# noc-lab/sac-expert

Hardware: NVIDIA B200
Metric: agent-updates/sec (higher is better)
Workload: dtype f32

## Files before the change

### sac_expert_b200/csrc/mlp_ws.cuh

```cuda
#pragma once
#include "tc_gemm.cuh"
#include "planes.cuh"

namespace saceo {

constexpr int WS_NEW = 16;
constexpr int WS_NEPI = WS_NEW * 32, WS_NT = WS_NEPI + 64;
constexpr int WS_NST = 3, WS_RING = WS_NST * WS_STAGE;
constexpr int WS_AUX = 49152;
constexpr int WS_PATCH1 = 32 * 32 * 4;
constexpr int WS_PATCH = WS_NEW * WS_PATCH1;
constexpr int WS_MAIN = WS_RING + WS_AUX + WS_PATCH;
constexpr int WS_BYTES = WS_MAIN + 1024 + 256;
constexpr int WS_RED = 40960;
constexpr int WS_MAXOUT = 36;
enum { WB_FULL = 0, WB_EMPTY = WS_NST, WB_XFULL = 2 * WS_NST, WB_XEMPTY, WB_D0, WB_D1, WB_AP  };

__device__ __forceinline__ void mbar_arrive(uint32_t bar) {
  asm volatile("mbarrier.arrive.shared::cta.b64 _, [%0];" ::"r"(bar) : "memory");
}
__device__ __forceinline__ void mbar_expect_tx(uint32_t bar, uint32_t bytes) {
  asm volatile("mbarrier.arrive.expect_tx.shared::cta.b64 _, [%0], %1;" ::"r"(bar), "r"(bytes) : "memory");
}
__device__ __forceinline__ void bulk_g2s(uint32_t dst, const void* src, uint32_t bytes, uint32_t bar) {
  asm volatile("cp.async.bulk.shared::cluster.global.mbarrier::complete_tx::bytes [%0], [%1], %2, [%3];"
               ::"r"(dst), "l"(src), "r"(bytes), "r"(bar) : "memory");
}
__device__ __forceinline__ void bulk_prefetch_l2(const void* src, uint32_t bytes) {
  asm volatile("cp.async.bulk.prefetch.L2.global [%0], %1;" ::"l"(src), "r"(bytes) : "memory");
}
__device__ __forceinline__ void epi_bar() { asm volatile("bar.sync 1, 512;" ::: "memory"); }
__device__ __forceinline__ uint64_t umma_desc_mn(uint32_t saddr) {
  return (uint64_t)((saddr >> 4) & 0x3FFF) | ((uint64_t)(4096 >> 4) << 16) | ((uint64_t)(1024 >> 4) << 32) |
         ((uint64_t)1 << 46) | ((uint64_t)2 << 61);
}
constexpr uint32_t WS_IDESC_FWD = (1u << 4) | (1u << 16) | ((uint32_t)(256 >> 3) << 17) | ((uint32_t)(128 >> 4) << 24);
constexpr uint32_t WS_IDESC_BWD = (1u << 4) | ((uint32_t)(128 >> 3) << 17) | ((uint32_t)(128 >> 4) << 24);

__global__ void k_planes_build(const float* __restrict__ theta, long long stride, uint8_t* __restrict__ img, int K0) {
  const int n0 = (K0 + 31) / 32, rows = n0 * 32 + 256;
  const int item = blockIdx.x * blockDim.x + threadIdx.x;
  if (item >= rows * 32) return;
  const int row = item >> 5, c8 = item & 31;
  const float* th = theta + (long long)blockIdx.y * stride;
  float x[8];
  if (row < n0 * 32) {
#pragma unroll
    for (int j = 0; j < 8; ++j) x[j] = row < K0 ? th[(long long)row * 256 + c8 * 8 + j] : 0.f;
  } else {
    const long long o = (long long)K0 * 256 + 256 + (long long)(row - n0 * 32) * 256 + c8 * 8;
#pragma unroll
    for (int j = 0; j < 8; ++j) x[j] = th[o + j];
  }
  uint4 hi, lo;
  split8<true>(x, hi, lo);
  uint8_t* dst = img + (long long)blockIdx.y * ws_image_bytes(K0) + ws_image_off(row, c8);
  *reinterpret_cast<uint4*>(dst) = hi;
  *reinterpret_cast<uint4*>(dst + 16384) = lo;
}

__device__ __forceinline__ uint32_t ws_pa(uint32_t patch, int r, int c) {
  return patch + (uint32_t)(r * 128 + ((((c >> 2) ^ (r & 7)) << 4) | ((c & 3) << 2)));
}
__device__ __forceinline__ void ws_store_rows(uint32_t patch, const uint32_t (&v)[32], float* __restrict__ G, int rbase,
                                              int rows, int col, int lane, uint32_t cs = 0, int q = 0) {
#pragma unroll
  for (int j = 0; j < 8; ++j) sts128(ws_pa(patch, lane, 4 * j), make_uint4(v[4 * j], v[4 * j + 1], v[4 * j + 2], v[4 * j + 3]));
  __syncwarp();
// ... 232 lines not shown
}
__device__ __forceinline__ void ws_split_f16(const uint32_t (&v)[32], float scale, uint32_t (&hi)[16], uint32_t (&lo)[16]) {
#pragma unroll
  for (int j = 0; j < 16; ++j) {
    const float x0 = __uint_as_float(v[2 * j]) * scale, x1 = __uint_as_float(v[2 * j + 1]) * scale;
    asm("cvt.rn.satfinite.f16x2.f32 %0, %1, %2;" : "=r"(hi[j]) : "f"(x1), "f"(x0));
    const float2 hf = __half22float2(*reinterpret_cast<const __half2*>(&hi[j]));
    asm("cvt.rn.satfinite.f16x2.f32 %0, %1, %2;" : "=r"(lo[j]) : "f"(x1 - hf.y), "f"(x0 - hf.x));
  }
}
template <int ACT>
__device__ __forceinline__ void ws_bias_act(uint32_t (&v)[32], uint32_t bias) {
#pragma unroll
  for (int j = 0; j < 8; ++j) {
    const float4 b = lds128(bias + j * 16);
    v[4 * j] = __float_as_uint(apply_act(ACT, __uint_as_float(v[4 * j]) + b.x));
    v[4 * j + 1] = __float_as_uint(apply_act(ACT, __uint_as_float(v[4 * j + 1]) + b.y));
    v[4 * j + 2] = __float_as_uint(apply_act(ACT, __uint_as_float(v[4 * j + 2]) + b.z));
    v[4 * j + 3] = __float_as_uint(apply_act(ACT, __uint_as_float(v[4 * j + 3]) + b.w));
  }
}
__device__ __forceinline__ void ws_bias_act_rt(int act, uint32_t (&v)[32], uint32_t bias) {
  if (act == ACT_RELU) ws_bias_act<ACT_RELU>(v, bias);
  else if (act == ACT_TANH) ws_bias_act<ACT_TANH>(v, bias);
  else ws_bias_act<ACT_ELU>(v, bias);
}
template <int ACT>
__device__ __forceinline__ void ws_mul_dact(uint32_t (&v)[32], const float (&aux)[32], float s) {
#pragma unroll
  for (int j = 0; j < 32; ++j) v[j] = __float_as_uint(__uint_as_float(v[j]) * s * dact_from_out(ACT, aux[j]));
}
__device__ __forceinline__ void ws_mul_dact_rt(int act, uint32_t (&v)[32], const float (&aux)[32], float s) {
  if (act == ACT_RELU) ws_mul_dact<ACT_RELU>(v, aux, s);
  else if (act == ACT_TANH) ws_mul_dact<ACT_TANH>(v, aux, s);
  else ws_mul_dact<ACT_ELU>(v, aux, s);
}
__device__ __forceinline__ float ws_row_scale(float bound) {
  if (!(bound > 0.f) || !(bound < 3.0e38f)) return 1.f;
  int e;
  frexpf(bound, &e);
  e = 10 - e;
  e = e > 120 ? 120 : (e < -120 ? -120 : e);
  return ldexpf(1.f, e);
}

struct FwdW {
  const float* X; int ldx; long long sXa, sXn;
  const float* theta; long long sTa, sTn;
  const uint8_t* planes; long long sPa, sPn;
  float* H1; float* H2; long long sHa, sHn;
  uint8_t* H1p; long long sQa, sQn;
  float* Out; int ldo; long long sOa, sOn;
  int rows, K0, nout, nnet, act0, act1;
  unsigned long long* dbg;
};
#define WS_STAMP(i) do { if (f.dbg && lane == 0) f.dbg[(size_t)(blockIdx.y * gridDim.x + blockIdx.x) * 16 + (i)] = gtime(); } while (0)

template <int NG>
__global__ void __launch_bounds__(WS_NT, 1) k_mlp_fwd_ws(FwdW f) {
  extern __shared__ uint8_t smem_raw[];
  const uint32_t sb = (smem_u32(smem_raw) + 1023u) & ~1023u;
  const uint32_t ring = sb, aux = sb + WS_RING, patch_base = aux + WS_AUX, bars = sb + WS_MAIN, tslot = bars + 8 * 16;
  auto bar = [&](int i) { return bars + 8u * (uint32_t)i; };
  const int z = blockIdx.y, agent = z / f.nnet, net = z - agent * f.nnet;
  const int row0 = blockIdx.x * TC_BM;
  const int warp = threadIdx.x >> 5, lane = threadIdx.x & 31;
  const int n0 = (f.K0 + 31) >> 5, nk64 = (f.K0 + 63) >> 6;

  if (threadIdx.x == 0) {
    for (int s = 0; s < 2 * WS_NST; ++s) mbar_init(bar(s), 1);
    mbar_init(bar(WB_XFULL), WS_NEW); mbar_init(bar(WB_XEMPTY), 1);
    mbar_init(bar(WB_D0), 1); mbar_init(bar(WB_D1), 1);
    for (int g = 0; g < 4; ++g) mbar_init(bar(WB_AP + g), 8);
    asm volatile("fence.mbarrier_init.release.cluster;" ::: "memory");
  }
  if (warp == WS_NEW + 1) {
    asm volatile("tcgen05.alloc.cta_group::1.sync.aligned.shared::cta.b32 [%0], %1;" ::"r"(tslot), "n"(512) : "memory");
    asm volatile("tcgen05.relinquish_alloc_permit.cta_group::1.sync.aligned;" ::: "memory");
  }
  asm volatile("tcgen05.fence::before_thread_sync;" ::: "memory");
  __syncthreads();
  asm volatile("tcgen05.fence::after_thread_sync;" ::: "memory");
  const uint32_t tmem = lds_u32(tslot);
  const uint32_t tP = tmem, tQ = tmem + 256;

  if (warp == WS_NEW) {
    if (lane == 0) {
      const uint8_t* img = f.planes + agent * f.sPa + net * f.sPn;
      const int total = n0 + 8;
      for (int it = 0; it < total; ++it) {
        const int s = it % WS_NST;
        mbar_wait(bar(WB_EMPTY + s), (uint32_t)(((it / WS_NST) & 1) ^ 1));
        mbar_expect_tx(bar(WB_FULL + s), WS_STAGE);
        bulk_g2s(ring + s * WS_STAGE, img + (long long)it * WS_STAGE, WS_STAGE, bar(WB_FULL + s));
        if (it == WS_NST - 1)
          for (int j = WS_NST; j < total; ++j) bulk_prefetch_l2(img + (long long)j * WS_STAGE, WS_STAGE);
      }
      WS_STAMP(11);
    }
  } else if (warp == WS_NEW + 1) {
    if (lane == 0) {
      int it = 0;
      for (int sl = 0; sl < nk64; ++sl) {
        mbar_wait(bar(WB_XFULL), (uint32_t)(sl & 1));
        asm volatile("tcgen05.fence::after_thread_sync;" ::: "memory");
        for (int hh = 0; hh < 2 && sl * 2 + hh < n0; ++hh, ++it) {
          const int s = it % WS_NST;
          mbar_wait(bar(WB_FULL + s), (uint32_t)((it / WS_NST) & 1));
          asm volatile("tcgen05.fence::after_thread_sync;" ::: "memory");
          const uint32_t st = ring + s * WS_STAGE;
#pragma unroll
          for (int kk = 0; kk < 2; ++kk) {
            const uint32_t ka = (uint32_t)(hh * 2 + kk) * 32, kb = (uint32_t)kk * 2048;
            umma_f16(tP, umma_desc(aux + ka), umma_desc_mn(st + kb), WS_IDESC_FWD, (it | kk) ? 1u : 0u);
            umma_f16(tP, umma_desc(aux + ka), umma_desc_mn(st + 16384 + kb), WS_IDESC_FWD, 1u);
            umma_f16(tP, umma_desc(aux + 16384 + ka), umma_desc_mn(st + kb), WS_IDESC_FWD, 1u);
          }
          umma_commit(bar(WB_EMPTY + s));
        }
        umma_commit(bar(WB_XEMPTY));
      }
      umma_commit(bar(WB_D0));
      WS_STAMP(8);
      for (int g = 0; g < 4; ++g) {
        mbar_wait(bar(WB_AP + g), 0);
        asm volatile("tcgen05.fence::after_thread_sync;" ::: "memory");
        if (g == 3) WS_STAMP(9);
        for (int tt = 0; tt < 2; ++tt, ++it) {
          const int t = 2 * g + tt, s = it % WS_NST;
          mbar_wait(bar(WB_FULL + s), (uint32_t)((it / WS_NST) & 1));
          asm volatile("tcgen05.fence::after_thread_sync;" ::: "memory");
          const uint32_t st = ring + s * WS_STAGE;
#pragma unroll
          for (int kk = 0; kk < 2; ++kk) {
            const uint32_t ta_hi = tP + 32 * t + 8 * kk, ta_lo = ta_hi + 16, kb = (uint32_t)kk * 2048;
            umma_f16_ts(tQ, ta_hi, umma_desc_mn(st + kb), WS_IDESC_FWD, (t | kk) ? 1u : 0u);
            umma_f16_ts(tQ, ta_hi, umma_desc_mn(st + 16384 + kb), WS_IDESC_FWD, 1u);
            umma_f16_ts(tQ, ta_lo, umma_desc_mn(st + kb), WS_IDESC_FWD, 1u);
          }
          umma_commit(bar(WB_EMPTY + s));
        }
      }
      umma_commit(bar(WB_D1));
      WS_STAMP(10);
    }
  } else {
    const int q = warp & 3, cg = warp >> 2;
    const uint32_t lane_addr = (uint32_t)(q * 32) << 16;
    const uint32_t patch = patch_base + (uint32_t)warp * WS_PATCH1;
    const int rbase = row0 + q * 32, grow = rbase + lane;
    const float* __restrict__ X = f.X + agent * f.sXa + net * f.sXn;
    const float* __restrict__ th = f.theta + agent * f.sTa + net * f.sTn;
    const long long ob0 = (long long)f.K0 * FW_H, oW1 = ob0 + FW_H, ob1 = oW1 + (long long)FW_H * FW_H,
                    oW2 = ob1 + FW_H, ob2 = oW2 + (long long)FW_H * f.nout;
    float* H1 = f.H1 ? f.H1 + agent * f.sHa + net * f.sHn : nullptr;
    float* H2 = f.H2 ? f.H2 + agent * f.sHa + net * f.sHn : nullptr;
    float* Out = f.Out + agent * f.sOa + net * f.sOn;
    if (warp == 0) WS_STAMP(0);
    const int np = (f.nout + 3) & ~3;
    const uint32_t cb0 = aux + WS_RED + 2048, cb1 = cb0 + 1024, cw2 = cb1 + 1024, cb2 = cw2 + 1024;
    if (threadIdx.x < FW_H) {
      const int t = threadIdx.x;
      asm volatile("st.shared.f32 [%0], %1;" ::"r"(cb0 + t * 4), "f"(__ldg(th + ob0 + t)) : "memory");
      asm volatile("st.shared.f32 [%0], %1;" ::"r"(cb1 + t * 4), "f"(__ldg(th + ob1 + t)) : "memory");
      if (f.nout == 1) asm volatile("st.shared.f32 [%0], %1;" ::"r"(cw2 + t * 4), "f"(__ldg(th + oW2 + t)) : "memory");
      if (t < f.nout) asm volatile("st.shared.f32 [%0], %1;" ::"r"(cb2 + t * 4), "f"(__ldg(th + ob2 + t)) : "memory");
    }
    {
      Slab<TC_BM, WS_NEPI> sx;
      sx.init(X, f.ldx, 1, row0, f.rows);
      for (int sl = 0; sl < nk64; ++sl) {
        sx.ld(sl * 64, f.K0);
        if (sl > 0) mbar_wait(bar(WB_XEMPTY), (uint32_t)((sl - 1) & 1));
        sx.template st<true>(aux, aux + 16384);
        asm volatile("fence.proxy.async.shared::cta;" ::: "memory");
        __syncwarp();
        if (lane == 0) mbar_arrive(bar(WB_XFULL));
      }
    }
    epi_bar();
    if (warp == 0) WS_STAMP(1);
    mbar_wait(bar(WB_D0), 0);
    asm volatile("tcgen05.fence::after_thread_sync;" ::: "memory");
    if (warp == 0) WS_STAMP(2);
#pragma unroll 1
    for (int c = 0; c < 2; ++c) {
      const int kg = 2 * c + (cg >> 1), col = kg * 64 + (cg & 1) * 32;
      uint32_t v[32];
      tmem_ld32(tP + lane_addr + (uint32_t)col, v);
      ws_bias_act_rt(f.act0, v, cb0 + col * 4);
      ws_split_store(tP + lane_addr + (uint32_t)col, v, 1.f);
      {
        asm volatile("tcgen05.wait::st.sync.aligned;" ::: "memory");
        asm volatile("tcgen05.fence::before_thread_sync;" ::: "memory");
        __syncwarp();
        if (lane == 0) mbar_arrive(bar(WB_AP + kg));
      }
      if (f.H1p) {
#pragma unroll
        for (int j = 0; j < 8; ++j) sts128(ws_pa(patch, lane, 4 * j), make_uint4(v[4 * j], v[4 * j + 1], v[4 * j + 2], v[4 * j + 3]));
        __syncwarp();
        ws_store_planes_p(patch, f.H1p + agent * f.sQa + net * f.sQn, rbase, f.rows, col, lane);
        __syncwarp();
      } else if (H1) { ws_store_rows(patch, v, H1, rbase, f.rows, col, lane); __syncwarp(); }
    }
    if (warp == 0) WS_STAMP(3);
    if (f.nout > 1 && threadIdx.x < FW_H) {
      float w2r[NG * 16];
      ws_load_wrow<NG * 16>(th + oW2, threadIdx.x, f.nout, w2r);
      ws_store_wrow<NG * 16>(aux, threadIdx.x, np, w2r);
    }
    epi_bar();
    if (warp == 0) WS_STAMP(4);
    mbar_wait(bar(WB_D1), 0);
    asm volatile("tcgen05.fence::after_thread_sync;" ::: "memory");
    if (warp == 0) WS_STAMP(5);
    float acc[NG * 16];
#pragma unroll
    for (int i = 0; i < NG * 16; ++i) acc[i] = 0.f;
    float qacc = 0.f;
    auto head_chunk = [&](uint32_t (&v)[32], int col) {
      if (f.nout == 1) {
#pragma unroll
        for (int j = 0; j < 8; ++j) {
          const float4 t4 = lds128(cw2 + (uint32_t)(col + 4 * j) * 4);
          qacc = fmaf(__uint_as_float(v[4 * j]), t4.x, qacc); qacc = fmaf(__uint_as_float(v[4 * j + 1]), t4.y, qacc);
          qacc = fmaf(__uint_as_float(v[4 * j + 2]), t4.z, qacc); qacc = fmaf(__uint_as_float(v[4 * j + 3]), t4.w, qacc);
        }
      } else {
#pragma unroll
        for (int jj = 0; jj < 32; ++jj) {
          const float h = __uint_as_float(v[jj]);
          const uint32_t wrow = aux + (uint32_t)((col + jj) * np) * 4;
#pragma unroll
          for (int g4 = 0; g4 < NG * 4; ++g4) {
            if (g4 * 4 < np) {
              const float4 w = lds128(wrow + g4 * 16);
              acc[4 * g4] = fmaf(h, w.x, acc[4 * g4]); acc[4 * g4 + 1] = fmaf(h, w.y, acc[4 * g4 + 1]);
              acc[4 * g4 + 2] = fmaf(h, w.z, acc[4 * g4 + 2]); acc[4 * g4 + 3] = fmaf(h, w.w, acc[4 * g4 + 3]);
            }
          }
        }
      }
    };
#pragma unroll 1
    for (int c = 0; c < 2; ++c) {
      const int col = cg * 64 + c * 32;
      uint32_t v[32];
      tmem_ld32(tQ + lane_addr + (uint32_t)col, v);
      ws_bias_act_rt(f.act1, v, cb1 + col * 4);
      if (H2) { ws_store_rows(patch, v, H2, rbase, f.rows, col, lane); __syncwarp(); }
      head_chunk(v, col);
    }
    if (warp == 0) WS_STAMP(6);
    const uint32_t red = aux + WS_RED;
    if (f.nout == 1) {
      if (cg > 0) asm volatile("st.shared.f32 [%0], %1;" ::"r"(red + (uint32_t)((cg - 1) * TC_BM + q * 32 + lane) * 4), "f"(qacc) : "memory");
      epi_bar();
      if (cg == 0 && grow < f.rows) {
        const uint32_t r = red + (uint32_t)(q * 32 + lane) * 4;
        Out[(long long)grow * f.ldo] = ((qacc + lds32(r)) + (lds32(r + TC_BM * 4) + lds32(r + 2 * TC_BM * 4))) + lds32(cb2);
      }
    } else {
#pragma unroll
      for (int r0 = 0; r0 < NG * 16; r0 += 32) {
        if (r0 < f.nout) {
          if (cg > 0) {
#pragma unroll
            for (int cc = 0; cc < 32; ++cc)
              if (r0 + cc < NG * 16) asm volatile("st.shared.f32 [%0], %1;" ::"r"(patch + (uint32_t)(lane * 32 + ((cc + lane) & 31)) * 4), "f"(acc[(r0 + cc) < NG * 16 ? r0 + cc : 0]) : "memory");
          }
          epi_bar();
          if (cg == 0 && grow < f.rows) {
#pragma unroll
            for (int cc = 0; cc < 32; ++cc) {
              if (r0 + cc < NG * 16 && r0 + cc < f.nout) {
                const uint32_t o = (uint32_t)(lane * 32 + ((cc + lane) & 31)) * 4;
                const float p1 = lds32(patch_base + (uint32_t)(warp + 4) * WS_PATCH1 + o), p2 = lds32(patch_base + (uint32_t)(warp + 8) * WS_PATCH1 + o),
                            p3 = lds32(patch_base + (uint32_t)(warp + 12) * WS_PATCH1 + o);
                Out[(long long)grow * f.ldo + r0 + cc] = ((acc[(r0 + cc) < NG * 16 ? r0 + cc : 0] + p1) + (p2 + p3)) + lds32(cb2 + (uint32_t)(r0 + cc) * 4);
              }
            }
          }
          if (r0 + 32 < f.nout) epi_bar();
        }
      }
    }
    if (warp == 0) WS_STAMP(7);
  }
  asm volatile("tcgen05.fence::before_thread_sync;" ::: "memory");
  __syncthreads();
  if (warp == WS_NEW + 1) {
    asm volatile("tcgen05.dealloc.cta_group::1.sync.aligned.b32 %0, %1;" ::"r"(tmem), "n"(512) : "memory");
  }
}

struct BwdW {
  const float* dOut; int ldd; long long sDa, sDn; int kout;
  const float* theta; long long sTa, sTn; int K0, nout;
  const uint8_t* planes; long long sPa, sPn;
  const float* H1; const float* H2; long long sHa, sHn;
  float* dH2; float* dH1;
  uint8_t* dH2p; long long sQa, sQn;
  uint8_t* dH1p;
  const uint8_t* H1p;
  float* dXa; int s_cols, a_cols; long long sXa, sXn;
  int rows, nnet, act0, act1;
  float* dbpart;
  unsigned long long* dbg;
};

template <int NG, int NA, int MODE>
__global__ void __launch_bounds__(WS_NT, 1) k_mlp_bwd_ws(BwdW f) {
  extern __shared__ uint8_t smem_raw[];
  const uint32_t sb = (smem_u32(smem_raw) + 1023u) & ~1023u;
  const uint32_t ring = sb, aux = sb + WS_RING, patch_base = aux + WS_AUX, bars = sb + WS_MAIN, tslot = bars + 8 * 16;
  const uint32_t cs2 = aux + WS_RED, cs1 = cs2 + 4096;
  auto bar = [&](int i) { return bars + 8u * (uint32_t)i; };
  const int z = blockIdx.y, agent = z / f.nnet, net = z - agent * f.nnet;
  const int row0 = blockIdx.x * TC_BM;
  const int warp = threadIdx.x >> 5, lane = threadIdx.x & 31;
  const int n0 = (f.K0 + 31) >> 5;

  if (threadIdx.x == 0) {
    for (int s = 0; s < 2 * WS_NST; ++s) mbar_init(bar(s), 1);
    mbar_init(bar(WB_D0), 1); mbar_init(bar(WB_D1), 1);
    for (int g = 0; g < 4; ++g) mbar_init(bar(WB_AP + g), 8);
    asm volatile("fence.mbarrier_init.release.cluster;" ::: "memory");
    asm volatile("st.shared.u32 [%0], %1;" ::"r"(aux + WS_RED - 256), "r"(0u) : "memory");
  }
  if (warp == WS_NEW + 1) {
    asm volatile("tcgen05.alloc.cta_group::1.sync.aligned.shared::cta.b32 [%0], %1;" ::"r"(tslot), "n"(512) : "memory");
    asm volatile("tcgen05.relinquish_alloc_permit.cta_group::1.sync.aligned;" ::: "memory");
  }
  asm volatile("tcgen05.fence::before_thread_sync;" ::: "memory");
  __syncthreads();
  asm volatile("tcgen05.fence::after_thread_sync;" ::: "memory");
  const uint32_t tmem = lds_u32(tslot);
  const uint32_t tP = tmem, tQ = tmem + 256;

  if (warp == WS_NEW) {
    if (lane == 0) {
      const uint8_t* w1 = f.planes + agent * f.sPa + net * f.sPn + (long long)n0 * WS_STAGE;
      for (int it = 0; it < 8; ++it) {
        const int h = it >> 2, sj = it & 3, s = it % WS_NST;
        mbar_wait(bar(WB_EMPTY + s), (uint32_t)(((it / WS_NST) & 1) ^ 1));
        mbar_expect_tx(bar(WB_FULL + s), WS_STAGE);
        for (int pl = 0; pl < 2; ++pl)
          for (int tt = 0; tt < 4; ++tt)
// ... 384 lines not shown
    epi_bar();
    if (threadIdx.x == 0) mbar_arrive(bar(2 * DW0_NST + 1));
  }
  if (warp == WS_NEW + 1) {
    if (lane == 0) {
      mbar_wait(bar(2 * DW0_NST + 1), 0);
      asm volatile("tcgen05.fence::after_thread_sync;" ::: "memory");
      for (int it = 0; it < nst; ++it) {
        const int s = it % DW0_NST;
        mbar_wait(bar(s), (uint32_t)((it / DW0_NST) & 1));
        asm volatile("tcgen05.fence::after_thread_sync;" ::: "memory");
        const uint32_t sa = xs + (uint32_t)it * DW0_XST, sbb = ring + s * WS_STAGE;
#pragma unroll
        for (int kk = 0; kk < 2; ++kk) {
          const uint32_t ko = (uint32_t)kk * 2048;
          const uint32_t a_hi = sa + ko, a_lo = a_hi + 4096, b_hi = sbb + ko, b_lo = b_hi + 16384, acc = (it | kk) ? 1u : 0u;
          umma_f16(tmem, umma_desc_mn(a_hi), umma_desc_mn(b_hi), DW_IDESC, acc);
          umma_f16(tmem, umma_desc_mn(a_hi), umma_desc_mn(b_lo), DW_IDESC, 1u);
          umma_f16(tmem, umma_desc_mn(a_lo), umma_desc_mn(b_hi), DW_IDESC, 1u);
        }
        umma_commit(bar(DW0_NST + s));
      }
      umma_commit(bar(2 * DW0_NST));
    }
  } else if (warp < WS_NEW) {
    const int q = warp & 3, cg = warp >> 2;
    if (q * 32 < f.in) {
      const uint32_t lane_addr = (uint32_t)(q * 32) << 16;
      const uint32_t patch = ring + (uint32_t)warp * WS_PATCH1;
      float* G = f.G + agent * f.sGa + net * f.sGn;
      mbar_wait(bar(2 * DW0_NST), 0);
      asm volatile("tcgen05.fence::after_thread_sync;" ::: "memory");
#pragma unroll 1
      for (int c = 0; c < 2; ++c) {
        const int col = cg * 64 + c * 32;
        uint32_t v[32];
        tmem_ld32(tmem + lane_addr + (uint32_t)col, v);
        ws_store_rows(patch, v, G, q * 32, f.in, col, lane);
        __syncwarp();
      }
    }
  }
  asm volatile("tcgen05.fence::before_thread_sync;" ::: "memory");
  __syncthreads();
  if (warp == WS_NEW + 1) {
    asm volatile("tcgen05.dealloc.cta_group::1.sync.aligned.b32 %0, %1;" ::"r"(tmem), "n"(256) : "memory");
  }
}
static inline bool dw0_planes_eligible(int in, int rows, int ldx, const float* X, long long sXa, long long sXn) {
  return in >= 1 && in <= 64 && ((rows + 31) >> 5) <= DW0_MAXST && (ldx % 4) == 0 && (reinterpret_cast<uintptr_t>(X) & 15) == 0 &&
         (sXa % 4) == 0 && (sXn % 4) == 0;
}

static inline cudaError_t mlp_ws_init() {
  static bool done_dev[64] = {};
  int dev_ = 0; cudaGetDevice(&dev_);
  bool& done = done_dev[dev_ & 63];
  if (done) return cudaSuccess;
  cudaError_t e;
#define WS_ATTR(K) e = cudaFuncSetAttribute(K, cudaFuncAttributeMaxDynamicSharedMemorySize, WS_BYTES); if (e) return e;
  WS_ATTR(k_mlp_fwd_ws<1>) WS_ATTR(k_mlp_fwd_ws<2>) WS_ATTR(k_mlp_fwd_ws<3>)
  WS_ATTR((k_mlp_bwd_ws<0, 0, 0>)) WS_ATTR((k_mlp_bwd_ws<0, 1, 0>)) WS_ATTR((k_mlp_bwd_ws<0, 2, 0>))
  WS_ATTR((k_mlp_bwd_ws<1, 0, 0>)) WS_ATTR((k_mlp_bwd_ws<2, 0, 0>)) WS_ATTR((k_mlp_bwd_ws<3, 0, 0>))
  WS_ATTR((k_mlp_bwd_ws<0, 0, 1>)) WS_ATTR((k_mlp_bwd_ws<1, 0, 1>)) WS_ATTR((k_mlp_bwd_ws<0, 1, 2>))
#undef WS_ATTR
  e = cudaFuncSetAttribute(k_dw_planes, cudaFuncAttributeMaxDynamicSharedMemorySize, DW_BYTES); if (e) return e;
  e = cudaFuncSetAttribute(k_dw0_planes, cudaFuncAttributeMaxDynamicSharedMemorySize, DW0_BYTES); if (e) return e;
  done = true;
  return cudaSuccess;
}
static inline bool mlp_fwd_ws_eligible(int h1, int h2, int nout, int K0, const float* theta, long long sTa, long long sTn) {
  return h1 == FW_H && h2 == FW_H && nout >= 1 && nout <= WS_MAXOUT && K0 >= 1 &&
         ((reinterpret_cast<uintptr_t>(theta) & 15) == 0) && ((sTa & 3) == 0) && ((sTn & 3) == 0);
}
static inline cudaError_t mlp_fwd_ws_launch(const FwdW& f, int nagents, cudaStream_t st) {
  dim3 grid((f.rows + TC_BM - 1) / TC_BM, nagents * f.nnet);
  if (f.nout <= 16) k_mlp_fwd_ws<1><<<grid, WS_NT, WS_BYTES, st>>>(f);
  else if (f.nout <= 32) k_mlp_fwd_ws<2><<<grid, WS_NT, WS_BYTES, st>>>(f);
  else k_mlp_fwd_ws<3><<<grid, WS_NT, WS_BYTES, st>>>(f);
  return cudaPeekAtLastError();
}
static inline bool mlp_bwd_ws_eligible(int h1, int h2, int kout, int nout, bool want_dxa, int a_cols, const float* theta, long long sTa,
                                       long long sTn) {
  if (!(h1 == FW_H && h2 == FW_H && kout >= 1 && kout <= WS_MAXOUT && kout <= nout)) return false;
  if (want_dxa && (kout != 1 || a_cols < 1 || a_cols > 32)) return false;
  return ((reinterpret_cast<uintptr_t>(theta) & 15) == 0) && ((sTa & 3) == 0) && ((sTn & 3) == 0);
}
static inline cudaError_t mlp_bwd_ws_launch(const BwdW& f, int nagents, cudaStream_t st) {
  dim3 grid((f.rows + TC_BM - 1) / TC_BM, nagents * f.nnet);
  const int ng = f.kout == 1 ? 0 : (f.kout + 15) / 16, na = f.dXa ? (f.a_cols + 15) / 16 : 0;
  const bool m1 = f.H1p && f.dH2p && f.dH1p && !f.dH2 && !f.dH1, m2 = f.H1p && !f.dH2p && !f.dH1p && !f.dH2 && !f.dH1;
  if (ng == 0 && na == 0 && m1) k_mlp_bwd_ws<0, 0, 1><<<grid, WS_NT, WS_BYTES, st>>>(f);
  else if (ng == 1 && na == 0 && m1) k_mlp_bwd_ws<1, 0, 1><<<grid, WS_NT, WS_BYTES, st>>>(f);
  else if (ng == 0 && na == 1 && m2) k_mlp_bwd_ws<0, 1, 2><<<grid, WS_NT, WS_BYTES, st>>>(f);
  else if (ng == 0 && na == 0) k_mlp_bwd_ws<0, 0, 0><<<grid, WS_NT, WS_BYTES, st>>>(f);
  else if (ng == 0 && na == 1) k_mlp_bwd_ws<0, 1, 0><<<grid, WS_NT, WS_BYTES, st>>>(f);
  else if (ng == 0) k_mlp_bwd_ws<0, 2, 0><<<grid, WS_NT, WS_BYTES, st>>>(f);
  else if (ng == 1) k_mlp_bwd_ws<1, 0, 0><<<grid, WS_NT, WS_BYTES, st>>>(f);
  else if (ng == 2) k_mlp_bwd_ws<2, 0, 0><<<grid, WS_NT, WS_BYTES, st>>>(f);
  else k_mlp_bwd_ws<3, 0, 0><<<grid, WS_NT, WS_BYTES, st>>>(f);
  return cudaPeekAtLastError();
}

}
```

Measured before the change: 127,000.

## Make forward warp-specialized MLP kernel persistent with cross-item prefetch and overlap

Turns the forward MLP kernel into a persistent kernel with one block per SM that loops over (agent, net, row-tile) work items. Barrier phases carry across items so the TMA producer and MMA warp can start the next item's weight planes and layer-1 GEMM while the epilogue warps finish the current one. Biases are double-buffered through cp.async, the W2 head matrix is staged into extra shared memory ahead of time, and the next item's X rows are prefetched into L2. This is meant to remove per-block launch, setup and TMEM-allocation cost and to hide load latency, at the price of more shared memory and more involved phase tracking.

```diff
diff --git a/sac_expert_b200/csrc/mlp_ws.cuh b/sac_expert_b200/csrc/mlp_ws.cuh
--- a/sac_expert_b200/csrc/mlp_ws.cuh
+++ b/sac_expert_b200/csrc/mlp_ws.cuh
@@ -13,7 +13,11 @@
 constexpr int WS_MAIN = WS_RING + WS_AUX + WS_PATCH;
 constexpr int WS_BYTES = WS_MAIN + 1024 + 256;
 constexpr int WS_RED = 40960;
+constexpr int WS_FWD_MAIN = WS_MAIN + 16384, WS_FWD_BYTES = WS_FWD_MAIN + 1024 + 256;
+constexpr int WS_CB1 = 36864;
+static_assert(WS_FWD_BYTES <= 232448, "fused forward kernel exceeds the per-block shared-memory limit");
 constexpr int WS_MAXOUT = 36;
+static_assert(WS_CB1 >= 256 * WS_MAXOUT * 4 && WS_CB1 + 3072 + WS_MAXOUT * 4 <= WS_RED, "constant buffer overlaps AUX neighbours");
 enum { WB_FULL = 0, WB_EMPTY = WS_NST, WB_XFULL = 2 * WS_NST, WB_XEMPTY, WB_D0, WB_D1, WB_AP  };
 
 __device__ __forceinline__ void mbar_arrive(uint32_t bar) {
@@ -352,20 +356,33 @@
   uint8_t* H1p; long long sQa, sQn;
   float* Out; int ldo; long long sOa, sOn;
   int rows, K0, nout, nnet, act0, act1;
+  int nitems;
   unsigned long long* dbg;
 };
-#define WS_STAMP(i) do { if (f.dbg && lane == 0) f.dbg[(size_t)(blockIdx.y * gridDim.x + blockIdx.x) * 16 + (i)] = gtime(); } while (0)
+#define WS_STAMP(i) do { if (f.dbg && lane == 0) f.dbg[(size_t)item * 16 + (i)] = gtime(); } while (0)
+__device__ __forceinline__ void cp_async4(uint32_t dst, const float* src) {
+  asm volatile("cp.async.ca.shared.global [%0], [%1], 4;" ::"r"(dst), "l"(src) : "memory");
+}
+__device__ __forceinline__ void cp_async_commit() { asm volatile("cp.async.commit_group;" ::: "memory"); }
+__device__ __forceinline__ void ws_x_prefetch(const float* __restrict__ X, int ldx, int row0, int rows, int K0) {
+  const int r = row0 + (int)(threadIdx.x & (TC_BM - 1));
+  if (r >= rows) return;
+  const float* p = X + (long long)r * ldx;
+  for (int c = (int)(threadIdx.x >> 7) * 32; c < K0; c += (WS_NEPI / TC_BM) * 32) asm volatile("prefetch.global.L2 [%0];" ::"l"(p + c));
+  if ((threadIdx.x >> 7) == 0) asm volatile("prefetch.global.L2 [%0];" ::"l"(p + K0 - 1));
+}
 
 template <int NG>
 __global__ void __launch_bounds__(WS_NT, 1) k_mlp_fwd_ws(FwdW f) {
+  constexpr bool W2OWN = NG == 1;
   extern __shared__ uint8_t smem_raw[];
   const uint32_t sb = (smem_u32(smem_raw) + 1023u) & ~1023u;
-  const uint32_t ring = sb, aux = sb + WS_RING, patch_base = aux + WS_AUX, bars = sb + WS_MAIN, tslot = bars + 8 * 16;
+  const uint32_t ring = sb, aux = sb + WS_RING, patch_base = aux + WS_AUX, bars = sb + WS_FWD_MAIN, tslot = bars + 8 * 16;
   auto bar = [&](int i) { return bars + 8u * (uint32_t)i; };
-  const int z = blockIdx.y, agent = z / f.nnet, net = z - agent * f.nnet;
-  const int row0 = blockIdx.x * TC_BM;
   const int warp = threadIdx.x >> 5, lane = threadIdx.x & 31;
-  const int n0 = (f.K0 + 31) >> 5, nk64 = (f.K0 + 63) >> 6;
+  const int n0 = (f.K0 + 31) >> 5, nk64 = (f.K0 + 63) >> 6, tiles = (f.rows + TC_BM - 1) / TC_BM;
+  const int ib = blockIdx.x, ie = f.nitems, is = gridDim.x;
+  const bool xearly = W2OWN && nk64 == 1;
 
   if (threadIdx.x == 0) {
     for (int s = 0; s < 2 * WS_NST; ++s) mbar_init(bar(s), 1);
@@ -386,207 +403,255 @@
 
   if (warp == WS_NEW) {
     if (lane == 0) {
-      const uint8_t* img = f.planes + agent * f.sPa + net * f.sPn;
       const int total = n0 + 8;
-      for (int it = 0; it < total; ++it) {
-        const int s = it % WS_NST;
-        mbar_wait(bar(WB_EMPTY + s), (uint32_t)(((it / WS_NST) & 1) ^ 1));
-        mbar_expect_tx(bar(WB_FULL + s), WS_STAGE);
-        bulk_g2s(ring + s * WS_STAGE, img + (long long)it * WS_STAGE, WS_STAGE, bar(WB_FULL + s));
-        if (it == WS_NST - 1)
-          for (int j = WS_NST; j < total; ++j) bulk_prefetch_l2(img + (long long)j * WS_STAGE, WS_STAGE);
-      }
-      WS_STAMP(11);
+      int it = 0;
+      for (int item = ib; item < ie; item += is) {
+        const int z = item / tiles, agent = z / f.nnet, net = z - agent * f.nnet;
+        const uint8_t* img = f.planes + agent * f.sPa + net * f.sPn;
+        for (int j = 0; j < total; ++j, ++it) {
+          const int s = it % WS_NST;
+          mbar_wait(bar(WB_EMPTY + s), (uint32_t)(((it / WS_NST) & 1) ^ 1));
+          mbar_expect_tx(bar(WB_FULL + s), WS_STAGE);
+          bulk_g2s(ring + s * WS_STAGE, img + (long long)j * WS_STAGE, WS_STAGE, bar(WB_FULL + s));
+          if (j == WS_NST - 1)
+            for (int jj = WS_NST; jj < total; ++jj) bulk_prefetch_l2(img + (long long)jj * WS_STAGE, WS_STAGE);
+        }
+        WS_STAMP(11);
+      }
     }
   } else if (warp == WS_NEW + 1) {
     if (lane == 0) {
-      int it = 0;
-      for (int sl = 0; sl < nk64; ++sl) {
-        mbar_wait(bar(WB_XFULL), (uint32_t)(sl & 1));
-        asm volatile("tcgen05.fence::after_thread_sync;" ::: "memory");
-        for (int hh = 0; hh < 2 && sl * 2 + hh < n0; ++hh, ++it) {
-          const int s = it % WS_NST;
-          mbar_wait(bar(WB_FULL + s), (uint32_t)((it / WS_NST) & 1));
+      int it = 0, gs = 0;
+      for (int item = ib, k = 0; item < ie; item += is, ++k) {
+        if (k > 0) {
+          mbar_wait(bar(WB_D1), (uint32_t)((k - 1) & 1));
           asm volatile("tcgen05.fence::after_thread_sync;" ::: "memory");
-          const uint32_t st = ring + s * WS_STAGE;
-#pragma unroll
-          for (int kk = 0; kk < 2; ++kk) {
-            const uint32_t ka = (uint32_t)(hh * 2 + kk) * 32, kb = (uint32_t)kk * 2048;
-            umma_f16(tP, umma_desc(aux + ka), umma_desc_mn(st + kb), WS_IDESC_FWD, (it | kk) ? 1u : 0u);
-            umma_f16(tP, umma_desc(aux + ka), umma_desc_mn(st + 16384 + kb), WS_IDESC_FWD, 1u);
-            umma_f16(tP, umma_desc(aux + 16384 + ka), umma_desc_mn(st + kb), WS_IDESC_FWD, 1u);
+        }
+        for (int sl = 0; sl < nk64; ++sl, ++gs) {
+          mbar_wait(bar(WB_XFULL), (uint32_t)(gs & 1));
+          asm volatile("tcgen05.fence::after_thread_sync;" ::: "memory");
+          for (int hh = 0; hh < 2 && sl * 2 + hh < n0; ++hh, ++it) {
+            const int s = it % WS_NST, lt = sl * 2 + hh;
+            mbar_wait(bar(WB_FULL + s), (uint32_t)((it / WS_NST) & 1));
+            asm volatile("tcgen05.fence::after_thread_sync;" ::: "memory");
+            const uint32_t st = ring + s * WS_STAGE;
+#pragma unroll
+            for (int kk = 0; kk < 2; ++kk) {
+              const uint32_t ka = (uint32_t)(hh * 2 + kk) * 32, kb = (uint32_t)kk * 2048;
+              umma_f16(tP, umma_desc(aux + ka), umma_desc_mn(st + kb), WS_IDESC_FWD, (lt | kk) ? 1u : 0u);
+              umma_f16(tP, umma_desc(aux + ka), umma_desc_mn(st + 16384 + kb), WS_IDESC_FWD, 1u);
+              umma_f16(tP, umma_desc(aux + 16384 + ka), umma_desc_mn(st + kb), WS_IDESC_FWD, 1u);
+            }
+            umma_commit(bar(WB_EMPTY + s));
           }
-          umma_commit(bar(WB_EMPTY + s));
-        }
-        umma_commit(bar(WB_XEMPTY));
-      }
-      umma_commit(bar(WB_D0));
-      WS_STAMP(8);
-      for (int g = 0; g < 4; ++g) {
-        mbar_wait(bar(WB_AP + g), 0);
-        asm volatile("tcgen05.fence::after_thread_sync;" ::: "memory");
-        if (g == 3) WS_STAMP(9);
-        for (int tt = 0; tt < 2; ++tt, ++it) {
-          const int t = 2 * g + tt, s = it % WS_NST;
-          mbar_wait(bar(WB_FULL + s), (uint32_t)((it / WS_NST) & 1));
+          umma_commit(bar(WB_XEMPTY));
+        }
+        umma_commit(bar(WB_D0));
+        WS_STAMP(8);
+        for (int g = 0; g < 4; ++g) {
+          mbar_wait(bar(WB_AP + g), (uint32_t)(k & 1));
           asm volatile("tcgen05.fence::after_thread_sync;" ::: "memory");
-          const uint32_t st = ring + s * WS_STAGE;
-#pragma unroll
-          for (int kk = 0; kk < 2; ++kk) {
-            const uint32_t ta_hi = tP + 32 * t + 8 * kk, ta_lo = ta_hi + 16, kb = (uint32_t)kk * 2048;
-            umma_f16_ts(tQ, ta_hi, umma_desc_mn(st + kb), WS_IDESC_FWD, (t | kk) ? 1u : 0u);
-            umma_f16_ts(tQ, ta_hi, umma_desc_mn(st + 16384 + kb), WS_IDESC_FWD, 1u);
-            umma_f16_ts(tQ, ta_lo, umma_desc_mn(st + kb), WS_IDESC_FWD, 1u);
+          if (g == 3) WS_STAMP(9);
+          for (int tt = 0; tt < 2; ++tt, ++it) {
+            const int t = 2 * g + tt, s = it % WS_NST;
+            mbar_wait(bar(WB_FULL + s), (uint32_t)((it / WS_NST) & 1));
+            asm volatile("tcgen05.fence::after_thread_sync;" ::: "memory");
+            const uint32_t st = ring + s * WS_STAGE;
+#pragma unroll
+            for (int kk = 0; kk < 2; ++kk) {
+              const uint32_t ta_hi = tP + 32 * t + 8 * kk, ta_lo = ta_hi + 16, kb = (uint32_t)kk * 2048;
+              umma_f16_ts(tQ, ta_hi, umma_desc_mn(st + kb), WS_IDESC_FWD, (t | kk) ? 1u : 0u);
+              umma_f16_ts(tQ, ta_hi, umma_desc_mn(st + 16384 + kb), WS_IDESC_FWD, 1u);
+              umma_f16_ts(tQ, ta_lo, umma_desc_mn(st + kb), WS_IDESC_FWD, 1u);
+            }
+            umma_commit(bar(WB_EMPTY + s));
           }
-          umma_commit(bar(WB_EMPTY + s));
-        }
-      }
-      umma_commit(bar(WB_D1));
-      WS_STAMP(10);
+        }
+        umma_commit(bar(WB_D1));
+        WS_STAMP(10);
+      }
     }
   } else {
     const int q = warp & 3, cg = warp >> 2;
     const uint32_t lane_addr = (uint32_t)(q * 32) << 16;
     const uint32_t patch = patch_base + (uint32_t)warp * WS_PATCH1;
-    const int rbase = row0 + q * 32, grow = rbase + lane;
-    const float* __restrict__ X = f.X + agent * f.sXa + net * f.sXn;
-    const float* __restrict__ th = f.theta + agent * f.sTa + net * f.sTn;
     const long long ob0 = (long long)f.K0 * FW_H, oW1 = ob0 + FW_H, ob1 = oW1 + (long long)FW_H * FW_H,
                     oW2 = ob1 + FW_H, ob2 = oW2 + (long long)FW_H * f.nout;
-    float* H1 = f.H1 ? f.H1 + agent * f.sHa + net * f.sHn : nullptr;
-    float* H2 = f.H2 ? f.H2 + agent * f.sHa + net * f.sHn : nullptr;
-    float* Out = f.Out + agent * f.sOa + net * f.sOn;
-    if (warp == 0) WS_STAMP(0);
     const int np = (f.nout + 3) & ~3;
-    const uint32_t cb0 = aux + WS_RED + 2048, cb1 = cb0 + 1024, cw2 = cb1 + 1024, cb2 = cw2 + 1024;
-    if (threadIdx.x < FW_H) {
+    auto cbuf = [&](int k_) { return (k_ & 1) ? aux + WS_CB1 : aux + WS_RED + 2048; };
+    const uint32_t w2s = W2OWN ? sb + WS_MAIN : aux;
+    auto stage_c = [&](int it_, uint32_t cb) {
+      const int z_ = it_ / tiles, a_ = z_ / f.nnet, n_ = z_ - a_ * f.nnet;
+      const float* th_ = f.theta + a_ * f.sTa + n_ * f.sTn;
       const int t = threadIdx.x;
-      asm volatile("st.shared.f32 [%0], %1;" ::"r"(cb0 + t * 4), "f"(__ldg(th + ob0 + t)) : "memory");
-      asm volatile("st.shared.f32 [%0], %1;" ::"r"(cb1 + t * 4), "f"(__ldg(th + ob1 + t)) : "memory");
-      if (f.nout == 1) asm volatile("st.shared.f32 [%0], %1;" ::"r"(cw2 + t * 4), "f"(__ldg(th + oW2 + t)) : "memory");
-      if (t < f.nout) asm volatile("st.shared.f32 [%0], %1;" ::"r"(cb2 + t * 4), "f"(__ldg(th + ob2 + t)) : "memory");
-    }
-    {
+      if (t < FW_H) {
+        cp_async4(cb + t * 4, th_ + ob0 + t);
+        cp_async4(cb + 1024 + t * 4, th_ + ob1 + t);
+        if (f.nout == 1) cp_async4(cb + 2048 + t * 4, th_ + oW2 + t);
+        if (t < f.nout) cp_async4(cb + 3072 + t * 4, th_ + ob2 + t);
+      }
+      cp_async_commit();
+    };
+    auto stage_w = [&](int it_) {
+      const int z_ = it_ / tiles, a_ = z_ / f.nnet, n_ = z_ - a_ * f.nnet;
+      const float* th_ = f.theta + a_ * f.sTa + n_ * f.sTn;
+      for (int e = threadIdx.x; e < FW_H * f.nout; e += WS_NEPI) { const int j = e / f.nout; cp_async4(w2s + (uint32_t)(j * np + e - j * f.nout) * 4, th_ + oW2 + e); }
+      cp_async_commit();
+    };
+    int gs = 0;
+    auto xconv = [&](int it_) {
+      const int z_ = it_ / tiles, a_ = z_ / f.nnet, n_ = z_ - a_ * f.nnet;
       Slab<TC_BM, WS_NEPI> sx;
-      sx.init(X, f.ldx, 1, row0, f.rows);
-      for (int sl = 0; sl < nk64; ++sl) {
+      sx.init(f.X + a_ * f.sXa + n_ * f.sXn, f.ldx, 1, (it_ - z_ * tiles) * TC_BM, f.rows);
+      for (int sl = 0; sl < nk64; ++sl, ++gs) {
         sx.ld(sl * 64, f.K0);
-        if (sl > 0) mbar_wait(bar(WB_XEMPTY), (uint32_t)((sl - 1) & 1));
+        if (gs > 0) mbar_wait(bar(WB_XEMPTY), (uint32_t)((gs - 1) & 1));
         sx.template st<true>(aux, aux + 16384);
         asm volatile("fence.proxy.async.shared::cta;" ::: "memory");
         __syncwarp();
         if (lane == 0) mbar_arrive(bar(WB_XFULL));
       }
-    }
-    epi_bar();
-    if (warp == 0) WS_STAMP(1);
-    mbar_wait(bar(WB_D0), 0);
-    asm volatile("tcgen05.fence::after_thread_sync;" ::: "memory");
-    if (warp == 0) WS_STAMP(2);
+    };
+    auto xprefetch = [&](int it_) {
+      const int z_ = it_ / tiles, a_ = z_ / f.nnet, n_ = z_ - a_ * f.nnet;
+      ws_x_prefetch(f.X + a_ * f.sXa + n_ * f.sXn, f.ldx, (it_ - z_ * tiles) * TC_BM, f.rows, f.K0);
+    };
+    if (W2OWN && f.nout > 1)
+      for (int e = threadIdx.x; e < FW_H * np; e += WS_NEPI) asm volatile("st.shared.f32 [%0], %1;" ::"r"(w2s + e * 4), "f"(0.f) : "memory");
+    if (ib < ie) {
+      stage_c(ib, cbuf(0));
+      if (W2OWN && f.nout > 1) stage_w(ib);
+      asm volatile("cp.async.wait_group 0;" ::: "memory");
+      xconv(ib);
+      epi_bar();
+    }
 #pragma unroll 1
-    for (int c = 0; c < 2; ++c) {
-      const int kg = 2 * c + (cg >> 1), col = kg * 64 + (cg & 1) * 32;
-      uint32_t v[32];
-      tmem_ld32(tP + lane_addr + (uint32_t)col, v);
-      ws_bias_act_rt(f.act0, v, cb0 + col * 4);
-      ws_split_store(tP + lane_addr + (uint32_t)col, v, 1.f);
-      {
-        asm volatile("tcgen05.wait::st.sync.aligned;" ::: "memory");
-        asm volatile("tcgen05.fence::before_thread_sync;" ::: "memory");
-        __syncwarp();
-        if (lane == 0) mbar_arrive(bar(WB_AP + kg));
-      }
-      if (f.H1p) {
-#pragma unroll
-        for (int j = 0; j < 8; ++j) sts128(ws_pa(patch, lane, 4 * j), make_uint4(v[4 * j], v[4 * j + 1], v[4 * j + 2], v[4 * j + 3]));
-        __syncwarp();
-        ws_store_planes_p(patch, f.H1p + agent * f.sQa + net * f.sQn, rbase, f.rows, col, lane);
-        __syncwarp();
-      } else if (H1) { ws_store_rows(patch, v, H1, rbase, f.rows, col, lane); __syncwarp(); }
-    }
-    if (warp == 0) WS_STAMP(3);
-    if (f.nout > 1 && threadIdx.x < FW_H) {
-      float w2r[NG * 16];
-      ws_load_wrow<NG * 16>(th + oW2, threadIdx.x, f.nout, w2r);
-      ws_store_wrow<NG * 16>(aux, threadIdx.x, np, w2r);
-    }
-    epi_bar();
-    if (warp == 0) WS_STAMP(4);
-    mbar_wait(bar(WB_D1), 0);
-    asm volatile("tcgen05.fence::after_thread_sync;" ::: "memory");
-    if (warp == 0) WS_STAMP(5);
-    float acc[NG * 16];
-#pragma unroll
-    for (int i = 0; i < NG * 16; ++i) acc[i] = 0.f;
-    float qacc = 0.f;
-    auto head_chunk = [&](uint32_t (&v)[32], int col) {
-      if (f.nout == 1) {
-#pragma unroll
-        for (int j = 0; j < 8; ++j) {
-          const float4 t4 = lds128(cw2 + (uint32_t)(col + 4 * j) * 4);
-          qacc = fmaf(__uint_as_float(v[4 * j]), t4.x, qacc); qacc = fmaf(__uint_as_float(v[4 * j + 1]), t4.y, qacc);
-          qacc = fmaf(__uint_as_float(v[4 * j + 2]), t4.z, qacc); qacc = fmaf(__uint_as_float(v[4 * j + 3]), t4.w, qacc);
-        }
-      } else {
-#pragma unroll
-        for (int jj = 0; jj < 32; ++jj) {
-          const float h = __uint_as_float(v[jj]);
-          const uint32_t wrow = aux + (uint32_t)((col + jj) * np) * 4;
-#pragma unroll
-          for (int g4 = 0; g4 < NG * 4; ++g4) {
-            if (g4 * 4 < np) {
-              const float4 w = lds128(wrow + g4 * 16);
-              acc[4 * g4] = fmaf(h, w.x, acc[4 * g4]); acc[4 * g4 + 1] = fmaf(h, w.y, acc[4 * g4 + 1]);
-              acc[4 * g4 + 2] = fmaf(h, w.z, acc[4 * g4 + 2]); acc[4 * g4 + 3] = fmaf(h, w.w, acc[4 * g4 + 3]);
-            }
+    for (int item = ib, k = 0; item < ie; item += is, ++k) {
+      const int z = item / tiles, agent = z / f.nnet, net = z - agent * f.nnet;
+      const int row0 = (item - z * tiles) * TC_BM, rbase = row0 + q * 32, grow = rbase + lane;
+      const long long hoff = agent * f.sHa + net * f.sHn;
+      const uint32_t cb0 = cbuf(k), cb1 = cb0 + 1024, cw2 = cb0 + 2048, cb2 = cb0 + 3072;
+      if (warp == 0) { WS_STAMP(0); if (f.dbg && lane == 0) f.dbg[(size_t)item * 16 + 15] = blockIdx.x; }
+      if (warp == 0) WS_STAMP(1);
+      if (item + is < ie) xprefetch(item + is);
+      mbar_wait(bar(WB_D0), (uint32_t)(k & 1));
+      asm volatile("tcgen05.fence::after_thread_sync;" ::: "memory");
+      if (warp == 0) WS_STAMP(2);
+#pragma unroll 1
+      for (int c = 0; c < 2; ++c) {
+        const int kg = 2 * c + (cg >> 1), col = kg * 64 + (cg & 1) * 32;
+        uint32_t v[32];
+        tmem_ld32(tP + lane_addr + (uint32_t)col, v);
+        ws_bias_act_rt(f.act0, v, cb0 + col * 4);
+        ws_split_store(tP + lane_addr + (uint32_t)col, v, 1.f);
+        {
+          asm volatile("tcgen05.wait::st.sync.aligned;" ::: "memory");
+          asm volatile("tcgen05.fence::before_thread_sync;" ::: "memory");
+          __syncwarp();
+          if (lane == 0) mbar_arrive(bar(WB_AP + kg));
+        }
+        if (f.H1p) {
+#pragma unroll
+          for (int j = 0; j < 8; ++j) sts128(ws_pa(patch, lane, 4 * j), make_uint4(v[4 * j], v[4 * j + 1], v[4 * j + 2], v[4 * j + 3]));
+          __syncwarp();
+          ws_store_planes_p(patch, f.H1p + agent * f.sQa + net * f.sQn, rbase, f.rows, col, lane);
+          __syncwarp();
+        } else if (f.H1) { ws_store_rows(patch, v, f.H1 + hoff, rbase, f.rows, col, lane); __syncwarp(); }
+      }
+      if (warp == 0) WS_STAMP(3);
+      if (xearly) {
+        if (item + is < ie) xconv(item + is);
+      } else if (!W2OWN && threadIdx.x < FW_H) {
+        float w2r[NG * 16];
+        ws_load_wrow<NG * 16>(f.theta + agent * f.sTa + net * f.sTn + oW2, threadIdx.x, f.nout, w2r);
+        ws_store_wrow<NG * 16>(w2s, threadIdx.x, np, w2r);
+      }
+      asm volatile("cp.async.wait_group 0;" ::: "memory");
+      epi_bar();
+      if (item + is < ie) stage_c(item + is, cbuf(k + 1));
+      if (warp == 0) WS_STAMP(4);
+      mbar_wait(bar(WB_D1), (uint32_t)(k & 1));
+      asm volatile("tcgen05.fence::after_thread_sync;" ::: "memory");
+      if (warp == 0) WS_STAMP(5);
+      float acc[NG * 16];
+#pragma unroll
+      for (int i = 0; i < NG * 16; ++i) acc[i] = 0.f;
+      float qacc = 0.f;
+      auto head_chunk = [&](uint32_t (&v)[32], int col) {
+        if (f.nout == 1) {
+#pragma unroll
+          for (int j = 0; j < 8; ++j) {
+            const float4 t4 = lds128(cw2 + (uint32_t)(col + 4 * j) * 4);
+            qacc = fmaf(__uint_as_float(v[4 * j]), t4.x, qacc); qacc = fmaf(__uint_as_float(v[4 * j + 1]), t4.y, qacc);
+            qacc = fmaf(__uint_as_float(v[4 * j + 2]), t4.z, qacc); qacc = fmaf(__uint_as_float(v[4 * j + 3]), t4.w, qacc);
           }
-        }
-      }
-    };
-#pragma unroll 1
-    for (int c = 0; c < 2; ++c) {
-      const int col = cg * 64 + c * 32;
-      uint32_t v[32];
-      tmem_ld32(tQ + lane_addr + (uint32_t)col, v);
-      ws_bias_act_rt(f.act1, v, cb1 + col * 4);
-      if (H2) { ws_store_rows(patch, v, H2, rbase, f.rows, col, lane); __syncwarp(); }
-      head_chunk(v, col);
-    }
-    if (warp == 0) WS_STAMP(6);
-    const uint32_t red = aux + WS_RED;
-    if (f.nout == 1) {
-      if (cg > 0) asm volatile("st.shared.f32 [%0], %1;" ::"r"(red + (uint32_t)((cg - 1) * TC_BM + q * 32 + lane) * 4), "f"(qacc) : "memory");
-      epi_bar();
-      if (cg == 0 && grow < f.rows) {
-        const uint32_t r = red + (uint32_t)(q * 32 + lane) * 4;
-        Out[(long long)grow * f.ldo] = ((qacc + lds32(r)) + (lds32(r + TC_BM * 4) + lds32(r + 2 * TC_BM * 4))) + lds32(cb2);
-      }
-    } else {
-#pragma unroll
-      for (int r0 = 0; r0 < NG * 16; r0 += 32) {
-        if (r0 < f.nout) {
-          if (cg > 0) {
-#pragma unroll
-            for (int cc = 0; cc < 32; ++cc)
-              if (r0 + cc < NG * 16) asm volatile("st.shared.f32 [%0], %1;" ::"r"(patch + (uint32_t)(lane * 32 + ((cc + lane) & 31)) * 4), "f"(acc[(r0 + cc) < NG * 16 ? r0 + cc : 0]) : "memory");
-          }
-          epi_bar();
-          if (cg == 0 && grow < f.rows) {
-#pragma unroll
-            for (int cc = 0; cc < 32; ++cc) {
-              if (r0 + cc < NG * 16 && r0 + cc < f.nout) {
-                const uint32_t o = (uint32_t)(lane * 32 + ((cc + lane) & 31)) * 4;
-                const float p1 = lds32(patch_base + (uint32_t)(warp + 4) * WS_PATCH1 + o), p2 = lds32(patch_base + (uint32_t)(warp + 8) * WS_PATCH1 + o),
-                            p3 = lds32(patch_base + (uint32_t)(warp + 12) * WS_PATCH1 + o);
-                Out[(long long)grow * f.ldo + r0 + cc] = ((acc[(r0 + cc) < NG * 16 ? r0 + cc : 0] + p1) + (p2 + p3)) + lds32(cb2 + (uint32_t)(r0 + cc) * 4);
+        } else {
+#pragma unroll
+          for (int jj = 0; jj < 32; ++jj) {
+            const float h = __uint_as_float(v[jj]);
+            const uint32_t wrow = w2s + (uint32_t)((col + jj) * np) * 4;
+#pragma unroll
+            for (int g4 = 0; g4 < NG * 4; ++g4) {
+              if (g4 * 4 < np) {
+                const float4 w = lds128(wrow + g4 * 16);
+                acc[4 * g4] = fmaf(h, w.x, acc[4 * g4]); acc[4 * g4 + 1] = fmaf(h, w.y, acc[4 * g4 + 1]);
+                acc[4 * g4 + 2] = fmaf(h, w.z, acc[4 * g4 + 2]); acc[4 * g4 + 3] = fmaf(h, w.w, acc[4 * g4 + 3]);
               }
             }
           }
-          if (r0 + 32 < f.nout) epi_bar();
-        }
-      }
-    }
-    if (warp == 0) WS_STAMP(7);
+        }
+      };
+#pragma unroll 1
+      for (int c = 0; c < 2; ++c) {
+        const int col = cg * 64 + c * 32;
+        uint32_t v[32];
+        tmem_ld32(tQ + lane_addr + (uint32_t)col, v);
+        ws_bias_act_rt(f.act1, v, cb1 + col * 4);
+        if (f.H2) { ws_store_rows(patch, v, f.H2 + hoff, rbase, f.rows, col, lane); __syncwarp(); }
+        head_chunk(v, col);
+      }
+      if (warp == 0) WS_STAMP(6);
+      asm volatile("cp.async.wait_group 0;" ::: "memory");
+      const uint32_t red = aux + WS_RED;
+      if (f.nout == 1) {
+        if (cg > 0) asm volatile("st.shared.f32 [%0], %1;" ::"r"(red + (uint32_t)((cg - 1) * TC_BM + q * 32 + lane) * 4), "f"(qacc) : "memory");
+        epi_bar();
+        if (cg == 0 && grow < f.rows) {
+          const uint32_t r = red + (uint32_t)(q * 32 + lane) * 4;
+          f.Out[agent * f.sOa + net * f.sOn + (long long)grow * f.ldo] = ((qacc + lds32(r)) + (lds32(r + TC_BM * 4) + lds32(r + 2 * TC_BM * 4))) + lds32(cb2);
+        }
+      } else {
+#pragma unroll
+        for (int r0 = 0; r0 < NG * 16; r0 += 32) {
+          if (r0 < f.nout) {
+            if (cg > 0) {
+#pragma unroll
+              for (int cc = 0; cc < 32; ++cc)
+                if (r0 + cc < NG * 16) asm volatile("st.shared.f32 [%0], %1;" ::"r"(patch + (uint32_t)(lane * 32 + ((cc + lane) & 31)) * 4), "f"(acc[(r0 + cc) < NG * 16 ? r0 + cc : 0]) : "memory");
+            }
+            epi_bar();
+            if (cg == 0 && grow < f.rows) {
+#pragma unroll
+              for (int cc = 0; cc < 32; ++cc) {
+                if (r0 + cc < NG * 16 && r0 + cc < f.nout) {
+                  const uint32_t o = (uint32_t)(lane * 32 + ((cc + lane) & 31)) * 4;
+                  const float p1 = lds32(patch_base + (uint32_t)(warp + 4) * WS_PATCH1 + o), p2 = lds32(patch_base + (uint32_t)(warp + 8) * WS_PATCH1 + o),
+                              p3 = lds32(patch_base + (uint32_t)(warp + 12) * WS_PATCH1 + o);
+                  f.Out[agent * f.sOa + net * f.sOn + (long long)grow * f.ldo + r0 + cc] = ((acc[(r0 + cc) < NG * 16 ? r0 + cc : 0] + p1) + (p2 + p3)) + lds32(cb2 + (uint32_t)(r0 + cc) * 4);
+                }
+              }
+            }
+            if (r0 + 32 < f.nout) epi_bar();
+          }
+        }
+      }
+      if (f.nout > 1) {
+        epi_bar();
+        if (W2OWN && item + is < ie) stage_w(item + is);
+      }
+      if (warp == 0) WS_STAMP(7);
+      if (!xearly && item + is < ie) xconv(item + is);
+    }
   }
   asm volatile("tcgen05.fence::before_thread_sync;" ::: "memory");
   __syncthreads();
@@ -595,6 +660,8 @@
   }
 }
 
+#undef WS_STAMP
+#define WS_STAMP(i) do { if (f.dbg && lane == 0) f.dbg[(size_t)(blockIdx.y * gridDim.x + blockIdx.x) * 16 + (i)] = gtime(); } while (0)
 struct BwdW {
   const float* dOut; int ldd; long long sDa, sDn; int kout;
   const float* theta; long long sTa, sTn; int K0, nout;
@@ -1085,6 +1152,7 @@
          (sXa % 4) == 0 && (sXn % 4) == 0;
 }
 
+static int g_ws_nsm[64] = {};
 static inline cudaError_t mlp_ws_init() {
   static bool done_dev[64] = {};
   int dev_ = 0; cudaGetDevice(&dev_);
@@ -1092,13 +1160,16 @@
   if (done) return cudaSuccess;
   cudaError_t e;
 #define WS_ATTR(K) e = cudaFuncSetAttribute(K, cudaFuncAttributeMaxDynamicSharedMemorySize, WS_BYTES); if (e) return e;
-  WS_ATTR(k_mlp_fwd_ws<1>) WS_ATTR(k_mlp_fwd_ws<2>) WS_ATTR(k_mlp_fwd_ws<3>)
+  e = cudaFuncSetAttribute(k_mlp_fwd_ws<1>, cudaFuncAttributeMaxDynamicSharedMemorySize, WS_FWD_BYTES); if (e) return e;
+  e = cudaFuncSetAttribute(k_mlp_fwd_ws<2>, cudaFuncAttributeMaxDynamicSharedMemorySize, WS_FWD_BYTES); if (e) return e;
+  e = cudaFuncSetAttribute(k_mlp_fwd_ws<3>, cudaFuncAttributeMaxDynamicSharedMemorySize, WS_FWD_BYTES); if (e) return e;
   WS_ATTR((k_mlp_bwd_ws<0, 0, 0>)) WS_ATTR((k_mlp_bwd_ws<0, 1, 0>)) WS_ATTR((k_mlp_bwd_ws<0, 2, 0>))
   WS_ATTR((k_mlp_bwd_ws<1, 0, 0>)) WS_ATTR((k_mlp_bwd_ws<2, 0, 0>)) WS_ATTR((k_mlp_bwd_ws<3, 0, 0>))
   WS_ATTR((k_mlp_bwd_ws<0, 0, 1>)) WS_ATTR((k_mlp_bwd_ws<1, 0, 1>)) WS_ATTR((k_mlp_bwd_ws<0, 1, 2>))
 #undef WS_ATTR
   e = cudaFuncSetAttribute(k_dw_planes, cudaFuncAttributeMaxDynamicSharedMemorySize, DW_BYTES); if (e) return e;
   e = cudaFuncSetAttribute(k_dw0_planes, cudaFuncAttributeMaxDynamicSharedMemorySize, DW0_BYTES); if (e) return e;
+  e = cudaDeviceGetAttribute(&g_ws_nsm[dev_ & 63], cudaDevAttrMultiProcessorCount, dev_); if (e) return e;
   done = true;
   return cudaSuccess;
 }
@@ -1106,11 +1177,15 @@
   return h1 == FW_H && h2 == FW_H && nout >= 1 && nout <= WS_MAXOUT && K0 >= 1 &&
          ((reinterpret_cast<uintptr_t>(theta) & 15) == 0) && ((sTa & 3) == 0) && ((sTn & 3) == 0);
 }
-static inline cudaError_t mlp_fwd_ws_launch(const FwdW& f, int nagents, cudaStream_t st) {
-  dim3 grid((f.rows + TC_BM - 1) / TC_BM, nagents * f.nnet);
-  if (f.nout <= 16) k_mlp_fwd_ws<1><<<grid, WS_NT, WS_BYTES, st>>>(f);
-  else if (f.nout <= 32) k_mlp_fwd_ws<2><<<grid, WS_NT, WS_BYTES, st>>>(f);
-  else k_mlp_fwd_ws<3><<<grid, WS_NT, WS_BYTES, st>>>(f);
+static inline cudaError_t mlp_fwd_ws_launch(FwdW f, int nagents, cudaStream_t st) {
+  f.nitems = nagents * f.nnet * ((f.rows + TC_BM - 1) / TC_BM);
+  if (f.nitems <= 0) return cudaSuccess;
+  int dev_ = 0; cudaGetDevice(&dev_);
+  const int nsm = g_ws_nsm[dev_ & 63] > 0 ? g_ws_nsm[dev_ & 63] : 1;
+  const dim3 grid(f.nitems < nsm ? f.nitems : nsm);
+  if (f.nout <= 16) k_mlp_fwd_ws<1><<<grid, WS_NT, WS_FWD_BYTES, st>>>(f);
+  else if (f.nout <= 32) k_mlp_fwd_ws<2><<<grid, WS_NT, WS_FWD_BYTES, st>>>(f);
+  else k_mlp_fwd_ws<3><<<grid, WS_NT, WS_FWD_BYTES, st>>>(f);
   return cudaPeekAtLastError();
 }
 static inline bool mlp_bwd_ws_eligible(int h1, int h2, int kout, int nout, bool want_dxa, int a_cols, const float* theta, long long sTa,
```

Result: faster. 129,900 (median of 6 runs) (+2.3%).
